# yutongwangBIT/multi_orbslam3

Measured on AMD Instinct MI355X. Metric: tracking+localBA frames/sec (aggregate over agents; 1 agent per GPU), higher is better.
Workload: dtype u8/int32 (ORB front-end, Hamming), f64 (local BA)

## Files before the change

### include/orbgpu.h

```cpp
#ifndef ORBGPU_H_
#define ORBGPU_H_

#include <stdint.h>

#ifdef __cplusplus
extern "C" {
#endif

enum {
  ORBG_OK = 0,
  ORBG_EMPTY = -1,
  ORBG_BAD_ARG = -2,
  ORBG_CAP_EXCEEDED = -3,
  ORBG_HIP_ERROR = -4,
  ORBG_NO_DEVICE = -5,
  ORBG_INTERNAL = -6
};

enum {
  LBA_APPLIED = 0,
  LBA_ABORTED_BEFORE_OPT = 1,
  LBA_REJECTED_OUTLIERS = 2
};

// ... 609 lines not shown
int lba_solve(const lba_problem* p, const volatile int32_t* stop_flag, lba_result* r);
int lba_solve_b(const lba_problem* p, const volatile uint8_t* stop_bool, lba_result* r);

typedef struct lba_handle lba_handle;
int lba_create(int device, int cap_poses, int cap_points, int cap_edges, lba_handle** out);
int lba_destroy(lba_handle* h);
int lba_solve_h(lba_handle* h, const lba_problem* p, const volatile int32_t* stop_flag, lba_result* r);
int lba_solve_hb(lba_handle* h, const lba_problem* p, const volatile uint8_t* stop_bool, lba_result* r);
int lba_solve_async(lba_handle* h, const lba_problem* problem, const volatile int32_t* stop_flag, lba_result* result);
int lba_solve_async_b(lba_handle* h, const lba_problem* problem, const volatile uint8_t* stop_bool, lba_result* result);
int lba_wait(lba_handle* h, double* solve_ms );
int lba_set_profiling(lba_handle* h, int on, int reset);
int lba_get_solver_stats(lba_handle* h, double* sum_ms, int64_t* n_brackets, int32_t* n_unknowns, int32_t* matrix_core);
int lba_event_overhead(lba_handle* h, int reps, float* ms);
int lba_get_watchdog_count(lba_handle* h, int64_t* n_timeouts);


typedef struct pose_opt_problem {
  int32_t n;
  const float* Xw;
  const float* u;
  const float* v;
  const float* ur;
  const float* inv_sigma2;
  float fx, fy, cx, cy, bf;
  float Tcw[16];
  int32_t device;
  const orbg_camera_rig* rig;
} pose_opt_problem;

// ... 43 lines not shown
```

### multi_orbslam3_amd/_capi.py

```python
import ctypes as C
import os

import numpy as np

_HERE = os.path.dirname(os.path.abspath(__file__))
LIB_PATH = os.environ.get("ORBG_LIB") or os.path.join(_HERE, "liborbgpu.so")

ORBG_OK, ORBG_EMPTY, ORBG_BAD_ARG, ORBG_CAP_EXCEEDED, ORBG_HIP_ERROR, ORBG_NO_DEVICE, ORBG_INTERNAL = 0, -1, -2, -3, -4, -5, -6
LBA_APPLIED, LBA_ABORTED_BEFORE_OPT, LBA_REJECTED_OUTLIERS = 0, 1, 2
GRID_COLS, GRID_ROWS = 64, 48

u8p = C.POINTER(C.c_uint8)
i32p = C.POINTER(C.c_int32)
u32p = C.POINTER(C.c_uint32)
f32p = C.POINTER(C.c_float)
f64p = C.POINTER(C.c_double)

KEYPOINT_DTYPE = np.dtype([("x", "<f4"), ("y", "<f4"), ("size", "<f4"), ("angle", "<f4"),
                           ("response", "<f4"), ("octave", "<i4")])
EDGE_DTYPE = np.dtype([("pose", "<i4"), ("point", "<i4"), ("u", "<f4"), ("v", "<f4"), ("ur", "<f4"),
                       ("inv_sigma2", "<f4")])
assert KEYPOINT_DTYPE.itemsize == 24 and EDGE_DTYPE.itemsize == 24


# ... 240 lines not shown


EXPORTED_SYMBOLS = [
    "orbx_create", "orbx_destroy", "orbx_get_tables", "orbx_extract", "orbx_extract_stereo",
    "orbx_extract_stereo_dev", "orbx_get_level", "orbx_get_level_bordered", "orbx_get_candidates", "orbx_stereo_match",
    "orbm_frame_create", "orbm_frame_destroy", "orbm_frame_upload", "orbm_frame_from_extractor", "orbx_frame_stereo_dev", "orbx_frame_stereo", "orbx_frame_stereo_dev_submit", "orbx_frame_stereo_dev_wait", "orbx_frame_stereo_submit", "orbx_frame_stereo_wait", "orbx_set_frame_outputs",
    "orbm_frame_get_grid", "orbm_hamming_matrix", "orbm_hamming_best2", "orbm_is_in_frustum",
    "orbm_search_by_projection_mps", "orbm_is_in_frustum_rig", "orbm_search_by_projection_mps_rig", "orbm_search_by_projection_frame_rig", "orbm_search_by_bow_rig", "orbx_fisheye_stereo_matches", "orbm_map_create", "orbm_map_destroy", "orbm_map_upload",
    "orbm_search_local_points", "orbm_search_local_points_vis", "orbm_search_by_projection_frame", "orbm_search_by_bow",
    "orbm_search_by_projection_sim3", "orbm_search_by_bow_kf",
    "orbv_vocab_create", "orbv_vocab_destroy", "orbv_text_load", "orbv_text_view", "orbv_text_free", "orbv_vocab_from_text", "orbv_transform", "orbv_transform_frame", "orbv_bow_assemble",
    "orbm_distinctive_descriptors", "orbv_score_l1", "orbk_wire_bytes", "orbk_pack_frame", "orbk_frame_from_wire",
    "orbm_frame_download",
    "lba_solve", "lba_create", "lba_destroy", "lba_solve_h", "lba_solve_async", "lba_wait", "pose_optimize",
    "lba_solve_b", "lba_solve_hb", "lba_solve_async_b",
    "lba_set_profiling", "lba_get_solver_stats", "lba_event_overhead", "lba_get_watchdog_count",
    "orbd_database_create", "orbd_database_destroy", "orbd_detect_n_best_candidates",
    "orbx_set_stream", "orbm_frame_set_stream", "orbm_map_set_stream", "lba_set_stream", "orbv_vocab_set_stream", "orbd_database_set_stream",
    "pose_opt_set_stream", "orbx_get_ctor_timeline", "orbm_map_set_observations", "orbm_search_by_projection_reloc", "orbm_search_by_projection_reloc_cam", "orbm_search_by_projection_sim3_cam", "orbm_lastview_create", "orbm_lastview_destroy", "orbm_lastview_upload",
    "orbm_search_by_projection_frame_resident", "orbg_quiesce", "orbg_set_wait_policy", "orbg_get_wait_policy",
    "orbx_frame_mono", "orbx_frame_mono_dev", "orbx_frame_mono_submit", "orbx_frame_mono_dev_submit", "orbx_frame_mono_wait",
    "orbx_set_frame_outputs_un", "orbx_undistort_points",
    "orbx_frame_rgbd", "orbx_frame_rgbd_dev", "orbx_frame_rgbd_submit", "orbx_frame_rgbd_dev_submit", "orbx_frame_rgbd_wait",
    "orbx_depth_at_points",
    "orbm_sim3_create", "orbm_sim3_destroy", "orbm_sim3_set_stream", "orbm_sim3_set_problem", "orbm_sim3_set_ransac_parameters",
    "orbm_sim3_ransac_iterations", "orbm_sim3_resolve_draws", "orbm_sim3_iterate", "orbm_sim3_solve_batch",
    "orbm_sim3_optimize", "orbm_sim3_optimize_batch",
    "orbm_create_new_points", "orbm_search_for_triangulation", "orbm_fuse", "orbm_search_for_initialization",
    "orbg_version", "orbg_strerror", "orbg_device_count", "orbx_get_timings", "orbx_event_overhead", "orbx_set_profile_interval", "orbx_set_profile_kernel", "orbx_get_fast_kernel_stats", "orbx_set_profiling",
]

# ... 61 lines not shown
```

### multi_orbslam3_amd/csrc/lba.hip

```cpp

#include <time.h>

#include <condition_variable>
#include <atomic>
#include <unistd.h>
#include <mutex>
#include <thread>

#include "common.hpp"
#include "wave.hpp"

#include <algorithm>
#include <cmath>
#include <limits>
#include <numeric>
#include <type_traits>

using namespace orbg;

#include "ldlt_mfma.hpp"
#include "ldlt_xcd.hpp"
#include "se3.hpp"

using namespace orbg_se3;

namespace {

#ifdef LBA_PROFILE
__device__ long long g_lba_prof[3][8 + 2 * 1020];
#define LBA_PROF_BEGIN(kern) const int lbp_k = (kern); const long long lbp_t0 = (long long)wall_clock64(); \
  if (threadIdx.x == 0 && blockIdx.x < 1020) g_lba_prof[lbp_k][8 + 2 * blockIdx.x] = lbp_t0
#define LBA_PROF_END() do { if (threadIdx.x == 0 && blockIdx.x < 1020) g_lba_prof[lbp_k][9 + 2 * blockIdx.x] = (long long)wall_clock64(); } while (0)
#define LBA_PROF_PHASE(block, slot) do { if (threadIdx.x == 0 && (int)blockIdx.x == (block)) g_lba_prof[lbp_k][slot] = (long long)wall_clock64() - lbp_t0; } while (0)
#else
#define LBA_PROF_BEGIN(kern) do { } while (0)
#define LBA_PROF_END() do { } while (0)
// ... 722 lines not shown
__device__ inline void inv3_sym(const double* h6, double lambda, double* o) {
  const double m0 = h6[0] + lambda, m1 = h6[1], m2 = h6[2], m4 = h6[3] + lambda, m5 = h6[4], m8 = h6[5] + lambda;
  const double c00 = m4 * m8 - m5 * m5, c01 = m5 * m2 - m1 * m8, c02 = m1 * m5 - m4 * m2;
  const double det = m0 * c00 + m1 * c01 + m2 * c02;
  const double id = 1.0 / det;
  o[0] = c00 * id; o[1] = c01 * id; o[2] = c02 * id;
  o[3] = o[1]; o[4] = (m0 * m8 - m2 * m2) * id; o[5] = (m2 * m1 - m0 * m5) * id;
  o[6] = o[2]; o[7] = o[5]; o[8] = (m0 * m4 - m1 * m1) * id;
}

struct PairItem { int ea, eb, l; };

constexpr int kSchurThreads = 256;

constexpr int kSortPfThreads = 64, kSortPfCap = 64;
template <int NT, int CAP, bool BY_EDGE = false>
__device__ __forceinline__ void sort_pf_block(int bid, int nL, const int* __restrict__ pf_start, int* __restrict__ pf_edges,
                                              int* __restrict__ pf_col, unsigned long long* __restrict__ lm_mask,
                                              const lba_edge* __restrict__ edges, const int* __restrict__ pose_col) {
  __shared__ int s_e[NT][CAP + 1];
  __shared__ int s_c[NT][CAP + 1];
  const int l = bid * NT + threadIdx.x;
  if (l >= nL) return;
  const int b0 = pf_start[l], cnt = pf_start[l + 1] - b0;
  unsigned long long m = 0;
  if (cnt <= CAP) {
    int* const se = s_e[threadIdx.x];
    int* const sc = s_c[threadIdx.x];
    for (int j = 0; j < cnt; j++) se[j] = pf_edges[b0 + j];
    for (int j = 0; j < cnt; j++) sc[j] = pose_col[edges[se[j]].pose];
    for (int a2 = 1; a2 < cnt; a2++) {
      const int e = se[a2], key = sc[a2];
      int b2 = a2 - 1;
      while (b2 >= 0 && (sc[b2] > key || (BY_EDGE && sc[b2] == key && se[b2] > e))) { se[b2 + 1] = se[b2]; sc[b2 + 1] = sc[b2]; b2--; }
      se[b2 + 1] = e; sc[b2 + 1] = key;
    }
    for (int j = 0; j < cnt; j++) { pf_edges[b0 + j] = se[j]; pf_col[b0 + j] = sc[j]; m |= 1ull << sc[j]; }
  } else {
    for (int a2 = b0 + 1; a2 < b0 + cnt; a2++) {
      const int e = pf_edges[a2], key = pose_col[edges[e].pose];
      int b2 = a2 - 1;
      while (b2 >= b0 && (pose_col[edges[pf_edges[b2]].pose] > key ||
                          (BY_EDGE && pose_col[edges[pf_edges[b2]].pose] == key && pf_edges[b2] > e))) { pf_edges[b2 + 1] = pf_edges[b2]; b2--; }
      pf_edges[b2 + 1] = e;
    }
    for (int j = b0; j < b0 + cnt; j++) { const int c = pose_col[edges[pf_edges[j]].pose]; pf_col[j] = c; m |= 1ull << c; }
  }
  lm_mask[l] = m;
}

__global__ __launch_bounds__(256) void k_csr_fill(int n_edges, const lba_edge* __restrict__ edges, const int* __restrict__ pose_col,
                                                 const int* __restrict__ point_col, int* __restrict__ cur_pt, int* __restrict__ cur_ps,
                                                 int* __restrict__ cur_pf, int* __restrict__ pt_edges, int* __restrict__ ps_edges,
                                                 int* __restrict__ pf_edges) {
  __shared__ int s_cnt[64], s_base[64];
  const int k = blockIdx.x * 256 + threadIdx.x;
  if (threadIdx.x < 64) s_cnt[threadIdx.x] = 0;
  __syncthreads();
  int lc = -1, pc = -1, my = 0;
  if (k < n_edges) {
    const lba_edge e = edges[k];
    lc = point_col[e.point]; pc = pose_col[e.pose];
    pt_edges[atomicAdd(&cur_pt[lc], 1)] = k;
    if (pc >= 0) { pf_edges[atomicAdd(&cur_pf[lc], 1)] = k; my = atomicAdd(&s_cnt[pc], 1); }
  }
  __syncthreads();
  if (threadIdx.x < 64 && s_cnt[threadIdx.x] > 0) s_base[threadIdx.x] = atomicAdd(&cur_ps[threadIdx.x], s_cnt[threadIdx.x]);
  __syncthreads();
  if (pc >= 0) ps_edges[s_base[pc] + my] = k;
}
constexpr int kPrep256Cap = 16, kPrep256Pad = 8, kPrep256Zero = 4;
constexpr int kCsrPoseCap = 4096, kCsrPtCap = 16;
__global__ __launch_bounds__(256) void k_csr_sort(int nP, int nL, const int* __restrict__ ps_start, int* __restrict__ ps_edges,
                                                 const int* __restrict__ pt_start, int* __restrict__ pt_edges,
                                                 const int* __restrict__ pf_start, int* __restrict__ pf_edges, int* __restrict__ pf_col,
                                                 unsigned long long* __restrict__ lm_mask, const lba_edge* __restrict__ edges,
                                                 const int* __restrict__ pose_col, int n_unknowns, double* __restrict__ St,
                                                 double* __restrict__ xzero, int n_zero) {
  __shared__ int s_pose[kCsrPoseCap];
  __shared__ int s_pt[256][kCsrPtCap + 1];
  int bid = (int)blockIdx.x;
  const int tid = threadIdx.x;
  if (bid < nP) {
    const int b0 = ps_start[bid], cnt = ps_start[bid + 1] - b0;
    int m = 1;
    while (m < cnt) m <<= 1;
    for (int i = tid; i < m; i += 256) s_pose[i] = i < cnt ? ps_edges[b0 + i] : 0x7FFFFFFF;
    __syncthreads();
    for (int k2 = 2; k2 <= m; k2 <<= 1)
      for (int j = k2 >> 1; j > 0; j >>= 1) {
        for (int i = tid; i < m; i += 256) {
          const int ixj = i ^ j;
          if (ixj > i) {
            const int a = s_pose[i], c = s_pose[ixj];
            const bool up = (i & k2) == 0;
            if ((a > c) == up) { s_pose[i] = c; s_pose[ixj] = a; }
          }
        }
        __syncthreads();
      }
    for (int i = tid; i < cnt; i += 256) ps_edges[b0 + i] = s_pose[i];
    return;
  }
  bid -= nP;
  const int n_pt_blocks = (nL + 255) / 256;
  if (bid < n_pt_blocks) {
    const int l = bid * 256 + tid;
    if (l < nL) {
      const int b0 = pt_start[l], cnt = pt_start[l + 1] - b0;
      if (cnt <= kCsrPtCap) {
        int* const se = s_pt[tid];
        for (int j = 0; j < cnt; j++) se[j] = pt_edges[b0 + j];
        for (int a2 = 1; a2 < cnt; a2++) {
          const int e = se[a2];
          int b2 = a2 - 1;
          while (b2 >= 0 && se[b2] > e) { se[b2 + 1] = se[b2]; b2--; }
          se[b2 + 1] = e;
        }
        for (int j = 0; j < cnt; j++) pt_edges[b0 + j] = se[j];
      } else {
        for (int a2 = b0 + 1; a2 < b0 + cnt; a2++) {
          const int e = pt_edges[a2];
          int b2 = a2 - 1;
          while (b2 >= b0 && pt_edges[b2] > e) { pt_edges[b2 + 1] = pt_edges[b2]; b2--; }
          pt_edges[b2 + 1] = e;
        }
      }
    }
    sort_pf_block<256, kCsrPtCap, true>(bid, nL, pf_start, pf_edges, pf_col, lm_mask, edges, pose_col);
    return;
  }
  bid -= n_pt_blocks;
  if (bid < kPrep256Pad) { if (St) ldltm::image_pad_range(n_unknowns, St, bid * 256 + tid, kPrep256Pad * 256); return; }
  bid -= kPrep256Pad;
  for (int i = bid * 256 + tid; i < n_zero; i += kPrep256Zero * 256) xzero[i] = 0.0;
}

template <class CamT>
__global__ __launch_bounds__(256) void k_errlin_prep(int n_errlin_blocks, int n_sort_blocks, int* __restrict__ pf_edges_w, int* __restrict__ pf_col_w,
                                                    const int* __restrict__ pf_start, unsigned long long* __restrict__ lm_mask,
                                                    int n_unknowns, double* __restrict__ St, double* __restrict__ xzero, int n_zero,
                                                    int nP, int n_edges, const lba_edge* __restrict__ edges, const PoseQ* __restrict__ poses,
                                               const double* __restrict__ points, CamT c, Huber hb, double* __restrict__ err,
                                               double* __restrict__ chi2, const int* __restrict__ pose_col,
                                               const int* __restrict__ point_col, double* __restrict__ EB,
                                               const int* __restrict__ ps_start, const int* __restrict__ ps_edges,
                                               double* __restrict__ Hpp, double* __restrict__ bp, double* __restrict__ partial,
                                               unsigned* __restrict__ ticket, const double* __restrict__ scale_partial, int n_scale_partial,
                                               const int* __restrict__ ok_flag, HostRec* __restrict__ rec, unsigned seq, int n_edge_blocks,
                                               int nL, const int* __restrict__ pt_start, const int* __restrict__ pt_edges,
// ... 480 lines not shown
  if (blockIdx.x == 0)
    finish_block(n_partial, partial, nP, nL, nullptr, bp, bl, Hpp, Hll, 0.0, nullptr, 0, 1, rec, lambda_init, lambda0_out);
  else
    build_items_block((int)blockIdx.x - 1, nP, nL, lm_mask, pf_start, pf_edges, pf_col, items, cap, pair_count);
}

}


struct StopRef {
  const volatile int32_t* i32 = nullptr;
  const volatile uint8_t* u8 = nullptr;
};
struct LbaSwitches {
  bool ldlt_wide = false;
  int ldlt_xcd = 1;
  bool ldlt_xcd_short_once = false;
  static LbaSwitches from_env() {
    LbaSwitches w;
    w.ldlt_wide = getenv("ORBG_LDLT_WIDE") != nullptr;
    if (const char* e = getenv("ORBG_LDLT_XCD")) { w.ldlt_xcd = !strcmp(e, "0") ? 0 : !strcmp(e, "safe") ? 2 : 1; w.ldlt_xcd_short_once = !strcmp(e, "short"); }
    return w;
  }
};
struct LinSet {
  DevBuf<double> EB, Hll, bl, Hpp, bp;
  int reserve(int NE, int nL, int nP) {
    int rc;
    if ((rc = EB.reserve(std::max<size_t>((size_t)NE * kEB, 1))) || (rc = Hll.reserve(std::max<size_t>(6 * (size_t)nL, 1))) ||
        (rc = bl.reserve(std::max<size_t>(3 * (size_t)nL, 1))) || (rc = Hpp.reserve(std::max<size_t>(21 * (size_t)nP, 1))) ||
        (rc = bp.reserve(std::max<size_t>(6 * (size_t)nP, 1))))
      return rc;
    return ORBG_OK;
  }
  void release() { EB.release(); Hll.release(); bl.release(); Hpp.release(); bp.release(); }
// ... 17 lines not shown
  DevBuf<double> d_err, d_chi2, d_partial, d_S, d_bs, d_x;
  LinSet lin[2];
  DevBuf<double> d_lambda0;
  DevBuf<double> d_wide;
  DevBuf<double> d_St, d_wfac;
  DevBuf<int> d_ok;
  PinnedBuf<HostRec> rec;
  unsigned rec_seq = 0;
  PinnedBuf<uint8_t> up_h, dl_h;
  DevBuf<uint8_t> up_d;
  DevBuf<double> d_scale_partial;
  DevBuf<unsigned> d_ticket;
  StreamSignal sig;
  std::vector<int> s_pose_deg, s_point_deg, s_pose_col, s_point_col, s_pf_deg, s_f1, s_f2, s_f3, s_fill, s_row_off, s_junk;
  std::vector<unsigned> s_cnt4;
  int prof_on = 0;
  hipEvent_t prof_ev[2] = {nullptr, nullptr};
  double prof_sum_ms = 0; long long prof_n = 0; int prof_n_unknowns = 0;
  long long prof_solves = 0;
  std::thread worker;
  std::mutex mu;
  std::condition_variable cv;
  std::atomic<bool> quit{false};
  std::atomic<int> job_state{0};
  const lba_problem* job_p = nullptr; StopRef job_stop; lba_result* job_r = nullptr;
  int job_status = ORBG_OK;
  double job_ms = 0;
};

extern "C" int lba_create(int device, int cap_poses, int cap_points, int cap_edges, lba_handle** out) {
// ... 87 lines not shown
  StopRef ref;
  int trials_done = 0;
  bool past_precheck = false;
  bool operator()() const {
    if (ref.u8) return *ref.u8 != 0;
    if (!ref.i32) return false;
    const int v = *ref.i32;
    if (v == INT32_MIN) return past_precheck;
    return v > 0 || (v < 0 && trials_done >= -v);
  }
};

struct Arena {
  PoseQ* poses; double* points;
  int *pose_col, *point_col, *pt_start, *ps_start, *pf_start;
  int *cur_pt, *cur_ps, *cur_pf;
  int *pt_edges, *ps_edges, *pf_edges, *pf_col;
  unsigned long long* lm_mask;
  int *pair_i1, *pair_i2, *pair_start;
  PairItem* items;
};
struct LbaStructure {
  int NP = 0, NX = 0, NE = 0;
  int nP = 0, nL = 0;
  int n = 0, n_zero = 0;
  int n_blocks_e = 0;
  int n_pairs_all = 0, item_cap = 0;
  int runs = 0;
  int n_right_edges = 0;
  std::vector<uint8_t> rig_secondary;
  bool dev_items = false;
  bool dev_lists = false;
  bool dev_csr = false;
  size_t o_poses = 0, o_points = 0, o_pose_col = 0, o_point_col = 0, o_pt_start = 0, o_ps_start = 0, o_pf_start = 0, o_cur_pt = 0,
         o_cur_ps = 0, o_cur_pf = 0, o_pt_edges = 0, o_ps_edges = 0, o_pf_edges = 0, o_pf_col = 0, o_lm_mask = 0, o_pair_i1 = 0,
         o_pair_i2 = 0, o_pair_start = 0, o_items = 0, o_end = 0;
  size_t off_a = 0;
  Arena H{};
  Arena at(uint8_t* B) const {
    auto I = [B](size_t o) { return reinterpret_cast<int*>(B + o); };
    return Arena{reinterpret_cast<PoseQ*>(B + o_poses), reinterpret_cast<double*>(B + o_points), I(o_pose_col), I(o_point_col),
                 I(o_pt_start), I(o_ps_start), I(o_pf_start), I(o_cur_pt), I(o_cur_ps), I(o_cur_pf), I(o_pt_edges), I(o_ps_edges),
                 I(o_pf_edges), I(o_pf_col), reinterpret_cast<unsigned long long*>(B + o_lm_mask), I(o_pair_i1), I(o_pair_i2),
                 I(o_pair_start), reinterpret_cast<PairItem*>(B + o_items)};
  }
};

struct LmState {
  int version = 0;
  int cur = 0;
  int ls = 0;
  bool err_valid = false;
  bool spec_ready = false;
  int fin_version = -1, solve_version = -1, exp_version = -1, exp_buf = -1;
  double lambda = -1, ni = 2, currentChi = 0;
  int nBad = 0;
  bool first_chi = true;
// ... 150 lines not shown
    return h->rec.h->ok == ldltx::kOkTimedOut ? kRcLdltTimedOut : ORBG_OK;
  }

  int edge_pass() {
    int rc;
    std::vector<int>& pose_deg = h->s_pose_deg; std::vector<int>& point_deg = h->s_point_deg;
    std::vector<int>& pf_raw = h->s_f3;
    pose_deg.assign(NP, 0); point_deg.assign(NX, 0); pf_raw.assign(NX, 0);
    if ((rc = h->edges_pin.reserve(std::max(NE, 1))) || (rc = h->d_edges.reserve(std::max(NE, 1)))) return rc;
    lba_edge* const edges = h->edges_pin.h;
    unsigned prev_pt = ~0u;
    if (NE < 65536) {
      std::vector<unsigned>& cnt4 = h->s_cnt4;
      cnt4.assign(4 * (size_t)NX, 0u);
      unsigned* const c4 = cnt4.data();
      int* const pd = pose_deg.data();
      const uint8_t* const fixed = p->pose_fixed;
      for (int k = 0; k < NE; k++) {
        const lba_edge e = p->edges[k];
        edges[k] = e;
        const unsigned ep = (unsigned)e.pose, ex = (unsigned)e.point;
        if (ep >= (unsigned)NP || ex >= (unsigned)NX) return ORBG_BAD_ARG;
        pd[ep]++;
        c4[(size_t)(k & 3) * NX + ex] += 1u + ((fixed[ep] ? 0u : 1u) << 16);
        runs += ex != prev_pt;
        prev_pt = ex;
      }
      int* const pdeg = point_deg.data(); int* const pfr = pf_raw.data();
      for (int i = 0; i < NX; i++) {
        const unsigned sum = c4[i] + c4[(size_t)NX + i] + c4[2 * (size_t)NX + i] + c4[3 * (size_t)NX + i];
        pdeg[i] = (int)(sum & 0xFFFFu); pfr[i] = (int)(sum >> 16);
      }
    } else {
      for (int k = 0; k < NE; k++) {
        const lba_edge e = p->edges[k];
        edges[k] = e;
        const unsigned ep = (unsigned)e.pose, ex = (unsigned)e.point;
        if (ep >= (unsigned)NP || ex >= (unsigned)NX) return ORBG_BAD_ARG;
        pose_deg[ep]++; point_deg[ex]++;
        pf_raw[ex] += p->pose_fixed[ep] ? 0 : 1;
// ... 14 lines not shown
    if (NE > 0) upload16(reinterpret_cast<const uint8_t*>(h->edges_pin.d), reinterpret_cast<uint8_t*>(h->d_edges.p), sizeof(lba_edge) * (size_t)NE, st);
    return ORBG_OK;
  }
  int layout() {
    constexpr bool kRig = std::is_same<CamT, CamRig>::value;
    const std::vector<int>& pose_deg = h->s_pose_deg; const std::vector<int>& point_deg = h->s_point_deg;
    const std::vector<int>& pf_raw = h->s_f3;
    std::vector<int>& pose_col_v = h->s_pose_col; std::vector<int>& point_col_v = h->s_point_col;
    pose_col_v.assign(NP, -1); point_col_v.assign(NX, -1);
    for (int i = 0; i < NP; i++) if (!p->pose_fixed[i] && pose_deg[i] > 0) pose_col_v[i] = nP++;
    for (int i = 0; i < NX; i++) if (point_deg[i] > 0) point_col_v[i] = nL++;
    n = 6 * nP; n_zero = n + 3 * nL;
    n_blocks_e = (NE + 255) / 256;
    std::vector<int>& pf_deg = h->s_pf_deg; std::vector<int>& pt_cnt = h->s_f1; std::vector<int>& ps_cnt = h->s_f2;
    pf_deg.assign(nL + 1, 0); pt_cnt.assign(nL + 1, 0); ps_cnt.assign(nP + 1, 0);
    int n_free_edges = 0;
    for (int i = 0; i < NX; i++) { const int lc = point_col_v[i]; if (lc >= 0) { pt_cnt[lc] = point_deg[i]; pf_deg[lc] = pf_raw[i]; } }
    for (int i = 0; i < NP; i++) { const int pc = pose_col_v[i]; if (pc >= 0) { ps_cnt[pc] = pose_deg[i]; n_free_edges += pose_deg[i]; } }
    size_t n_items = 0;
    for (int l = 0; l < nL; l++) n_items += (size_t)pf_deg[l] * (pf_deg[l] + 1) / 2;
    n_pairs_all = nP * (nP + 1) / 2;
    size_t off = 0;
    auto take = [&](size_t bytes) { const size_t o = off; off = (off + bytes + 63) & ~(size_t)63; return o; };
    o_poses = take(sizeof(PoseQ) * (size_t)NP); o_points = take(24 * (size_t)NX);
    o_pose_col = take(4 * (size_t)NP); o_point_col = take(4 * (size_t)NX); o_pt_start = take(4 * ((size_t)nL + 1));
    o_ps_start = take(4 * ((size_t)nP + 1)); o_pf_start = take(4 * ((size_t)nL + 1));
    o_cur_pt = take(4 * (size_t)nL); o_cur_ps = take(4 * (size_t)nP); o_cur_pf = take(4 * (size_t)nL);
    o_pt_edges = take(4 * (size_t)NE); o_ps_edges = take(4 * (size_t)n_free_edges);
    o_pf_edges = take(4 * (size_t)n_free_edges); o_pf_col = take(4 * (size_t)n_free_edges);
    int max_pose_edges = 1;
    for (int i = 0; i < nP; i++) max_pose_edges = std::max(max_pose_edges, ps_cnt[i]);
    item_cap = std::min(std::max(nL, 1), max_pose_edges);
    dev_items = nP >= 1 && nP <= 64 && (size_t)n_pairs_all * (size_t)item_cap * sizeof(PairItem) <= ((size_t)64 << 20);
    dev_lists = dev_items && nP >= 1 && ldltm::supports(6 * nP);
    dev_csr = dev_lists && NE > 0 && nL > 0 && max_pose_edges <= kCsrPoseCap && NE >= 16384 && !kRig;
    o_lm_mask = take(8 * (size_t)nL);
    o_pair_i1 = take(4 * (size_t)n_pairs_all); o_pair_i2 = take(4 * (size_t)n_pairs_all); o_pair_start = take(4 * ((size_t)n_pairs_all + 1));
    o_items = take(dev_items ? 0 : sizeof(PairItem) * n_items);
    o_end = off;
    off_a = dev_csr ? o_pt_edges : dev_lists ? o_pf_col : o_pf_edges;
    int rc;
    if ((rc = h->up_h.reserve(off + 64)) || (rc = h->up_d.reserve(off + 64))) return rc;
    H = at(h->up_h.h);
    return ORBG_OK;
  }
  void fill_lists() {
    constexpr bool kRig = std::is_same<CamT, CamRig>::value;
    const Arena A = H;
    const lba_edge* const edges = h->edges_pin.h;
    memcpy(A.pose_col, h->s_pose_col.data(), 4 * (size_t)NP);
    memcpy(A.point_col, h->s_point_col.data(), 4 * (size_t)NX);
    const std::vector<int>& pt_cnt = h->s_f1; const std::vector<int>& ps_cnt = h->s_f2; const std::vector<int>& pf_deg = h->s_pf_deg;
    A.pt_start[0] = 0; A.pf_start[0] = 0; A.ps_start[0] = 0;
    for (int i = 0; i < nL; i++) { A.pt_start[i + 1] = A.pt_start[i] + pt_cnt[i]; A.pf_start[i + 1] = A.pf_start[i] + pf_deg[i]; }
    for (int i = 0; i < nP; i++) A.ps_start[i + 1] = A.ps_start[i] + ps_cnt[i];
    if (dev_csr) {
      memcpy(A.cur_pt, A.pt_start, 4 * (size_t)nL); memcpy(A.cur_ps, A.ps_start, 4 * (size_t)nP); memcpy(A.cur_pf, A.pf_start, 4 * (size_t)nL);
      return;
    }
    std::vector<int>& f1 = h->s_f1; std::vector<int>& f2 = h->s_f2; std::vector<int>& f3 = h->s_f3;
    if (runs == nL && !kRig) {
      f2.assign(A.ps_start, A.ps_start + nP);
      f2.push_back(0);
      std::vector<int>& junk = h->s_junk;
      if ((int)junk.size() < NE + 1) junk.resize((size_t)NE + 1);
      int* const ps_base[2] = {junk.data(), A.ps_edges};
      int* const f2p = f2.data();
      int prev = -1, pt_pos = 0, pf_pos = 0;
      for (int k = 0; k < NE; k++) {
        const int ex = edges[k].point, lc = A.point_col[ex], pc = A.pose_col[edges[k].pose];
        const bool ch = ex != prev;
        prev = ex;
// ... 60 lines not shown
    if (use_wide && (rc = h->d_wide.reserve(2 * (size_t)n + 32))) return rc;
    if (use_mfma) {
      if ((rc = h->d_St.reserve(ldltm::tile_image_doubles(n))) || (rc = h->d_wfac.reserve(ldltm::wglob_doubles(ldltm::make_geo(n))))) return rc;
    }
    use_xcd = use_mfma && h->sw.ldlt_xcd != 0 && ldltx::pays(n);
    if (use_xcd && !h->ldlt_x.scr) {
      if ((rc = h->d_xscr.reserve(ldltx::scratch_doubles())) || (rc = h->d_xflags.reserve(ldltx::kFlagWords))) return rc;
      ORBG_HIP(hipMemsetAsync(h->d_xflags.p, 0, ldltx::kFlagWords * sizeof(unsigned), st));
      ORBG_HIP(hipMemsetAsync(h->d_xscr.p + ldltx::kGbOff, 0, (ldltx::kWOff - ldltx::kGbOff) * sizeof(double), st));
      h->ldlt_x.bind(h->d_xscr.p, h->d_xflags.p);
      static std::atomic<int> n_users{0};
      h->ldlt_x.pick = ((int)getpid() + n_users.fetch_add(1)) & 7;
    }
    n_blocks_u = (NP + NX + kUpdThreads - 1) / kUpdThreads;
    if ((rc = h->d_scale_partial.reserve(std::max(n_blocks_u, 1)))) return rc;
    if (!h->d_ticket.p) {
      if ((rc = h->d_ticket.reserve(4))) return rc;
      ORBG_HIP(hipMemsetAsync(h->d_ticket.p, 0, 4 * sizeof(unsigned), st));
    }
    size_t off = 0;
    auto take = [&](size_t bytes) { const size_t o = off; off = (off + bytes + 63) & ~(size_t)63; return o; };
    o_rposes = take(sizeof(PoseQ) * (size_t)NP); o_rpoints = take(24 * (size_t)NX); o_rflags = take((size_t)NE);
    o_rchi = take(r->edge_chi2 ? 8 * (size_t)NE : 0);
    if ((rc = h->dl_h.reserve(off + 64))) return rc;
    out.flags = h->dl_h.d + o_rflags;
    out.chi2 = r->edge_chi2 ? reinterpret_cast<double*>(h->dl_h.d + o_rchi) : (double*)nullptr;
    out.poses = reinterpret_cast<PoseQ*>(h->dl_h.d + o_rposes);
    out.points = reinterpret_cast<double*>(h->dl_h.d + o_rpoints);
    prof_this_solve = h->prof_on && (h->prof_solves++ & 3) == 0;
    return ORBG_OK;
  }

  int first_linearisation() {
    first2 = dev_lists && NE > 0 && nL > 0 && !stop();
    if (first2 || !stop()) {
      const int set = lm.ls ^ 1;
      if (first2) {
        if (dev_csr) {
          hipLaunchKernelGGL(k_csr_fill, dim3(n_blocks_e), dim3(256), 0, st, NE, d_edges, D.pose_col, D.point_col, D.cur_pt, D.cur_ps,
                             D.cur_pf, D.pt_edges, D.ps_edges, D.pf_edges);
          const int n_blocks_l = (nL + 255) / 256;
          hipLaunchKernelGGL(k_csr_sort, dim3(nP + n_blocks_l + kPrep256Pad + kPrep256Zero), dim3(256), 0, st, nP, nL, D.ps_start,
                             D.ps_edges, D.pt_start, D.pt_edges, D.pf_start, D.pf_edges, D.pf_col, D.lm_mask, d_edges, D.pose_col, n,
                             use_mfma ? h->d_St.p : (double*)nullptr, h->d_x.p, n_zero);
          errlin(lm.cur, set, false, LmIn{});
        } else {
          errlin_prep(lm.cur, set);
        }
        finish_items(set);
        lm.fin_version = lm.version;
      } else if (NE > 0) {
        errlin(lm.cur, set, false, LmIn{});
        finish_lambda_init(set);
        lm.fin_version = lm.version;
      }
      ORBG_HIP(hipGetLastError());
      lm.err_valid = true;
      lm.spec_ready = true;
    }
    if (first2) return ORBG_OK;
    if (dev_lists) {
      const int nsb = (nL + kSortPfThreads - 1) / kSortPfThreads;
      hipLaunchKernelGGL(k_prep, dim3(nsb + 32 + 8), dim3(kSortPfThreads), 0, st, nsb, nL, D.pf_start, D.pf_edges, D.pf_col, D.lm_mask,
// ... 28 lines not shown
          for (int j = b0; j < e0; j++) m |= 1ull << A.pf_col[j];
          A.lm_mask[l] = m;
        } else {
          for (int a2 = b0; a2 < e0; a2++) {
            const int ro = row_off[A.pf_col[a2]] + 1;
            for (int b2 = a2; b2 < e0; b2++) A.pair_start[ro + A.pf_col[b2]]++;
          }
        }
      }
    }
    for (int i1 = 0, id = 0; i1 < nP; i1++)
      for (int i2 = i1; i2 < nP; i2++, id++) { A.pair_i1[id] = i1; A.pair_i2[id] = i2; }
    int rc;
    if (dev_items) {
      if (stop()) return ORBG_OK;
      if (!dev_lists && (rc = upload_arena(h, off_a, o_pair_start, st))) return rc;
      if (nL > 0 && !first2)
        hipLaunchKernelGGL(k_build_items, dim3(n_pairs_all), dim3(256), 0, st, nP, nL, D.lm_mask, D.pf_start, D.pf_edges, D.pf_col,
                           h->d_items_dev.p, item_cap, h->d_pair_count.p);
      ORBG_HIP(hipGetLastError());
      return ORBG_OK;
    }
    for (int i = 0; i < n_pairs_all; i++) A.pair_start[i + 1] += A.pair_start[i];
    std::vector<int>& fill = h->s_fill;
    fill.assign(A.pair_start, A.pair_start + n_pairs_all);
    const std::vector<int>& row_off = h->s_row_off;
    for (int l = 0; l < nL; l++) {
      const int b0 = A.pf_start[l], e0 = A.pf_start[l + 1];
      for (int a2 = b0; a2 < e0; a2++) {
        const int ro = row_off[A.pf_col[a2]], ea = A.pf_edges[a2];
        for (int b2 = a2; b2 < e0; b2++) A.items[fill[ro + A.pf_col[b2]]++] = PairItem{ea, A.pf_edges[b2], l};
// ... 244 lines not shown

#ifdef LBA_PROFILE
extern "C" int lba_debug_prof(long long* out , int reset) {
  if (hipMemcpyFromSymbol(out, HIP_SYMBOL(g_lba_prof), sizeof(g_lba_prof)) != hipSuccess) return -1;
  if (reset) { static long long z[3][8 + 2 * 1020]; if (hipMemcpyToSymbol(HIP_SYMBOL(g_lba_prof), z, sizeof(z)) != hipSuccess) return -1; }
  return 0;
}
#endif

extern "C" int lba_get_watchdog_count(lba_handle* h, int64_t* n_timeouts) {
  if (!h || !n_timeouts) return ORBG_BAD_ARG;
  *n_timeouts = h->xcd_timeouts;
  return ORBG_OK;
}

extern "C" int lba_event_overhead(lba_handle* h, int reps, float* ms) {
  if (!h || !ms || reps < 1) return ORBG_BAD_ARG;
  int rc = select_device(h->device);
  if (rc) return rc;
  if ((rc = lba_set_profiling(h, h->prof_on, 0))) return rc;
  if (!h->prof_ev[0]) { ORBG_HIP(hipEventCreate(&h->prof_ev[0])); ORBG_HIP(hipEventCreate(&h->prof_ev[1])); }
  double acc = 0;
  for (int i = 0; i < reps; i++) {
    ORBG_HIP(hipEventRecord(h->prof_ev[0], h->stream));
    ORBG_HIP(hipEventRecord(h->prof_ev[1], h->stream));
    ORBG_HIP(hipStreamSynchronize(h->stream));
    float e = 0;
    ORBG_HIP(hipEventElapsedTime(&e, h->prof_ev[0], h->prof_ev[1]));
    acc += e;
  }
// ... 108 lines not shown
```

Baseline: 9059.

## Build LBA CSR edge lists deterministically via per-block pose bases instead of atomics+sort

Replaces the atomic-scatter CSR fill plus bitonic/insertion sort kernels with a single ordered kernel. Host counting now records per-256-edge-block pose counts and each point's first edge, so ps_edges are placed by wave ballot ranks and pt/pf edges are written as contiguous runs. This removes the sort passes and atomics and widens the device-CSR path to smaller problems (NE<65536, edges grouped by point), at the cost of extra host-side counting and a per-block×pose base table upload. Adds a debug API to read back the lists and an env switch to force host lists.

```diff
diff --git a/include/orbgpu.h b/include/orbgpu.h
--- a/include/orbgpu.h
+++ b/include/orbgpu.h
@@ -647,6 +647,13 @@
 int lba_get_solver_stats(lba_handle* h, double* sum_ms, int64_t* n_brackets, int32_t* n_unknowns, int32_t* matrix_core);
 int lba_event_overhead(lba_handle* h, int reps, float* ms);
 int lba_get_watchdog_count(lba_handle* h, int64_t* n_timeouts);
+typedef struct lba_lists_info {
+  int32_t struct_size;
+  int32_t n_free_poses, n_active_points, n_edges, n_free_edges;
+  int32_t device_filled;
+} lba_lists_info;
+int lba_debug_lists(lba_handle* h, lba_lists_info* info, int32_t* pt_start, int32_t* pt_edges, int32_t* ps_start, int32_t* ps_edges,
+                    int32_t* pf_start, int32_t* pf_edges);
 
 
 typedef struct pose_opt_problem {
diff --git a/multi_orbslam3_amd/_capi.py b/multi_orbslam3_amd/_capi.py
--- a/multi_orbslam3_amd/_capi.py
+++ b/multi_orbslam3_amd/_capi.py
@@ -278,7 +278,7 @@
     "orbm_frame_download",
     "lba_solve", "lba_create", "lba_destroy", "lba_solve_h", "lba_solve_async", "lba_wait", "pose_optimize",
     "lba_solve_b", "lba_solve_hb", "lba_solve_async_b",
-    "lba_set_profiling", "lba_get_solver_stats", "lba_event_overhead", "lba_get_watchdog_count",
+    "lba_set_profiling", "lba_get_solver_stats", "lba_event_overhead", "lba_get_watchdog_count", "lba_debug_lists",
     "orbd_database_create", "orbd_database_destroy", "orbd_detect_n_best_candidates",
     "orbx_set_stream", "orbm_frame_set_stream", "orbm_map_set_stream", "lba_set_stream", "orbv_vocab_set_stream", "orbd_database_set_stream",
     "pose_opt_set_stream", "orbx_get_ctor_timeline", "orbm_map_set_observations", "orbm_search_by_projection_reloc", "orbm_search_by_projection_reloc_cam", "orbm_search_by_projection_sim3_cam", "orbm_lastview_create", "orbm_lastview_destroy", "orbm_lastview_upload",
diff --git a/multi_orbslam3_amd/csrc/csr_blocks.hpp b/multi_orbslam3_amd/csrc/csr_blocks.hpp
--- /dev/null
+++ b/multi_orbslam3_amd/csrc/csr_blocks.hpp
@@ -0,0 +1,39 @@
+#pragma once
+#include <cstddef>
+
+namespace orbg {
+namespace csr {
+
+constexpr int kBlockEdges = 256;
+constexpr int kBlockShift = 8;
+
+inline int n_blocks(int n_edges) { return (n_edges + kBlockEdges - 1) / kBlockEdges; }
+inline size_t count_words(int n_edges, int n_poses) { return (size_t)n_blocks(n_edges) * (size_t)n_poses; }
+
+inline void count_edge(int k, unsigned pose, unsigned point, bool new_run, int n_poses, int n_points, int* blk_cnt, int* first_raw) {
+  blk_cnt[(size_t)(k >> kBlockShift) * n_poses + pose]++;
+  first_raw[new_run ? point : (unsigned)n_points] = k;
+}
+
+inline void block_bases(int n_blk, int n_poses, const int* blk_cnt, const int* pose_col, const int* ps_start, int* blk_base) {
+  for (int i = 0; i < n_poses; i++) {
+    const int pc = pose_col[i];
+    int run = pc >= 0 ? ps_start[pc] : 0;
+    for (int b = 0; b < n_blk; b++) {
+      const size_t at = (size_t)b * n_poses + i;
+      const int c = blk_cnt[at];
+      blk_base[at] = pc >= 0 ? run : c;
+      run += c;
+    }
+  }
+}
+
+inline void first_by_column(int n_points, const int* point_col, const int* first_raw, int* first_edge) {
+  for (int i = 0; i < n_points; i++) {
+    const int lc = point_col[i];
+    if (lc >= 0) first_edge[lc] = first_raw[i];
+  }
+}
+
+}
+}
diff --git a/multi_orbslam3_amd/csrc/lba.hip b/multi_orbslam3_amd/csrc/lba.hip
--- a/multi_orbslam3_amd/csrc/lba.hip
+++ b/multi_orbslam3_amd/csrc/lba.hip
@@ -20,6 +20,7 @@
 
 #include "ldlt_mfma.hpp"
 #include "ldlt_xcd.hpp"
+#include "csr_blocks.hpp"
 #include "se3.hpp"
 
 using namespace orbg_se3;
@@ -772,7 +773,7 @@
 constexpr int kSchurThreads = 256;
 
 constexpr int kSortPfThreads = 64, kSortPfCap = 64;
-template <int NT, int CAP, bool BY_EDGE = false>
+template <int NT, int CAP>
 __device__ __forceinline__ void sort_pf_block(int bid, int nL, const int* __restrict__ pf_start, int* __restrict__ pf_edges,
                                               int* __restrict__ pf_col, unsigned long long* __restrict__ lm_mask,
                                               const lba_edge* __restrict__ edges, const int* __restrict__ pose_col) {
@@ -790,7 +791,7 @@
     for (int a2 = 1; a2 < cnt; a2++) {
       const int e = se[a2], key = sc[a2];
       int b2 = a2 - 1;
-      while (b2 >= 0 && (sc[b2] > key || (BY_EDGE && sc[b2] == key && se[b2] > e))) { se[b2 + 1] = se[b2]; sc[b2 + 1] = sc[b2]; b2--; }
+      while (b2 >= 0 && sc[b2] > key) { se[b2 + 1] = se[b2]; sc[b2 + 1] = sc[b2]; b2--; }
       se[b2 + 1] = e; sc[b2 + 1] = key;
     }
     for (int j = 0; j < cnt; j++) { pf_edges[b0 + j] = se[j]; pf_col[b0 + j] = sc[j]; m |= 1ull << sc[j]; }
@@ -798,8 +799,7 @@
     for (int a2 = b0 + 1; a2 < b0 + cnt; a2++) {
       const int e = pf_edges[a2], key = pose_col[edges[e].pose];
       int b2 = a2 - 1;
-      while (b2 >= b0 && (pose_col[edges[pf_edges[b2]].pose] > key ||
-                          (BY_EDGE && pose_col[edges[pf_edges[b2]].pose] == key && pf_edges[b2] > e))) { pf_edges[b2 + 1] = pf_edges[b2]; b2--; }
+      while (b2 >= b0 && pose_col[edges[pf_edges[b2]].pose] > key) { pf_edges[b2 + 1] = pf_edges[b2]; b2--; }
       pf_edges[b2 + 1] = e;
     }
     for (int j = b0; j < b0 + cnt; j++) { const int c = pose_col[edges[pf_edges[j]].pose]; pf_col[j] = c; m |= 1ull << c; }
@@ -807,91 +807,49 @@
   lm_mask[l] = m;
 }
 
-__global__ __launch_bounds__(256) void k_csr_fill(int n_edges, const lba_edge* __restrict__ edges, const int* __restrict__ pose_col,
-                                                 const int* __restrict__ point_col, int* __restrict__ cur_pt, int* __restrict__ cur_ps,
-                                                 int* __restrict__ cur_pf, int* __restrict__ pt_edges, int* __restrict__ ps_edges,
-                                                 int* __restrict__ pf_edges) {
-  __shared__ int s_cnt[64], s_base[64];
-  const int k = blockIdx.x * 256 + threadIdx.x;
-  if (threadIdx.x < 64) s_cnt[threadIdx.x] = 0;
-  __syncthreads();
-  int lc = -1, pc = -1, my = 0;
-  if (k < n_edges) {
-    const lba_edge e = edges[k];
-    lc = point_col[e.point]; pc = pose_col[e.pose];
-    pt_edges[atomicAdd(&cur_pt[lc], 1)] = k;
-    if (pc >= 0) { pf_edges[atomicAdd(&cur_pf[lc], 1)] = k; my = atomicAdd(&s_cnt[pc], 1); }
-  }
-  __syncthreads();
-  if (threadIdx.x < 64 && s_cnt[threadIdx.x] > 0) s_base[threadIdx.x] = atomicAdd(&cur_ps[threadIdx.x], s_cnt[threadIdx.x]);
-  __syncthreads();
-  if (pc >= 0) ps_edges[s_base[pc] + my] = k;
-}
 constexpr int kPrep256Cap = 16, kPrep256Pad = 8, kPrep256Zero = 4;
-constexpr int kCsrPoseCap = 4096, kCsrPtCap = 16;
-__global__ __launch_bounds__(256) void k_csr_sort(int nP, int nL, const int* __restrict__ ps_start, int* __restrict__ ps_edges,
-                                                 const int* __restrict__ pt_start, int* __restrict__ pt_edges,
-                                                 const int* __restrict__ pf_start, int* __restrict__ pf_edges, int* __restrict__ pf_col,
-                                                 unsigned long long* __restrict__ lm_mask, const lba_edge* __restrict__ edges,
-                                                 const int* __restrict__ pose_col, int n_unknowns, double* __restrict__ St,
-                                                 double* __restrict__ xzero, int n_zero) {
-  __shared__ int s_pose[kCsrPoseCap];
-  __shared__ int s_pt[256][kCsrPtCap + 1];
-  int bid = (int)blockIdx.x;
-  const int tid = threadIdx.x;
-  if (bid < nP) {
-    const int b0 = ps_start[bid], cnt = ps_start[bid + 1] - b0;
-    int m = 1;
-    while (m < cnt) m <<= 1;
-    for (int i = tid; i < m; i += 256) s_pose[i] = i < cnt ? ps_edges[b0 + i] : 0x7FFFFFFF;
+__global__ __launch_bounds__(256) void k_csr_ordered(int n_edges, int n_edge_blocks, int n_poses, int nL, const lba_edge* __restrict__ edges,
+                                                    const int* __restrict__ pose_col, const int* __restrict__ blk_base,
+                                                    const int* __restrict__ first_edge, const int* __restrict__ pt_start,
+                                                    const int* __restrict__ pf_start, int* __restrict__ pt_edges,
+                                                    int* __restrict__ ps_edges, int* __restrict__ pf_edges ,
+                                                    unsigned* __restrict__ ticket) {
+  __shared__ int s_wcnt[4][64];
+  const int bid = (int)blockIdx.x, tid = (int)threadIdx.x, lane = tid & 63, wv = tid >> 6;
+  if (bid < n_edge_blocks) {
+    if (bid == 0 && tid < 4) ticket[tid] = 0u;
+    s_wcnt[wv][lane] = 0;
+    const int k = bid * 256 + tid;
+    int pose = -1, pc = -1;
+    if (k < n_edges) { pose = edges[k].pose; pc = pose_col[pose]; }
+    int rank = 0;
+    unsigned long long todo = __ballot(pc >= 0);
+    while (todo) {
+      const int leader = __ffsll((long long)todo) - 1;
+      const int lp = __builtin_amdgcn_readlane(pc, leader);
+      const unsigned long long same = __ballot(pc == lp);
+      if (pc == lp) {
+        rank = __popcll(same & ((1ull << lane) - 1ull));
+        if (lane == leader) s_wcnt[wv][lp] = __popcll(same);
+      }
+      todo &= ~same;
+    }
     __syncthreads();
-    for (int k2 = 2; k2 <= m; k2 <<= 1)
-      for (int j = k2 >> 1; j > 0; j >>= 1) {
-        for (int i = tid; i < m; i += 256) {
-          const int ixj = i ^ j;
-          if (ixj > i) {
-            const int a = s_pose[i], c = s_pose[ixj];
-            const bool up = (i & k2) == 0;
-            if ((a > c) == up) { s_pose[i] = c; s_pose[ixj] = a; }
-          }
-        }
-        __syncthreads();
-      }
-    for (int i = tid; i < cnt; i += 256) ps_edges[b0 + i] = s_pose[i];
+    if (pc >= 0) {
+      int before = 0;
+      for (int w = 0; w < wv; w++) before += s_wcnt[w][pc];
+      ps_edges[blk_base[(size_t)bid * n_poses + pose] + before + rank] = k;
+    }
     return;
   }
-  bid -= nP;
-  const int n_pt_blocks = (nL + 255) / 256;
-  if (bid < n_pt_blocks) {
-    const int l = bid * 256 + tid;
-    if (l < nL) {
-      const int b0 = pt_start[l], cnt = pt_start[l + 1] - b0;
-      if (cnt <= kCsrPtCap) {
-        int* const se = s_pt[tid];
-        for (int j = 0; j < cnt; j++) se[j] = pt_edges[b0 + j];
-        for (int a2 = 1; a2 < cnt; a2++) {
-          const int e = se[a2];
-          int b2 = a2 - 1;
-          while (b2 >= 0 && se[b2] > e) { se[b2 + 1] = se[b2]; b2--; }
-          se[b2 + 1] = e;
-        }
-        for (int j = 0; j < cnt; j++) pt_edges[b0 + j] = se[j];
-      } else {
-        for (int a2 = b0 + 1; a2 < b0 + cnt; a2++) {
-          const int e = pt_edges[a2];
-          int b2 = a2 - 1;
-          while (b2 >= b0 && pt_edges[b2] > e) { pt_edges[b2 + 1] = pt_edges[b2]; b2--; }
-          pt_edges[b2 + 1] = e;
-        }
-      }
-    }
-    sort_pf_block<256, kCsrPtCap, true>(bid, nL, pf_start, pf_edges, pf_col, lm_mask, edges, pose_col);
-    return;
-  }
-  bid -= n_pt_blocks;
-  if (bid < kPrep256Pad) { if (St) ldltm::image_pad_range(n_unknowns, St, bid * 256 + tid, kPrep256Pad * 256); return; }
-  bid -= kPrep256Pad;
-  for (int i = bid * 256 + tid; i < n_zero; i += kPrep256Zero * 256) xzero[i] = 0.0;
+  const int l = (bid - n_edge_blocks) * 256 + tid;
+  if (l >= nL) return;
+  const int k0 = first_edge[l], b0 = pt_start[l], cnt = pt_start[l + 1] - b0;
+  int q = pf_start[l];
+  for (int j = 0; j < cnt; j++) {
+    pt_edges[b0 + j] = k0 + j;
+    if (pf_edges && pose_col[edges[k0 + j].pose] >= 0) pf_edges[q++] = k0 + j;
+  }
 }
 
 template <class CamT>
@@ -1402,11 +1360,13 @@
 };
 struct LbaSwitches {
   bool ldlt_wide = false;
+  bool host_lists = false;
   int ldlt_xcd = 1;
   bool ldlt_xcd_short_once = false;
   static LbaSwitches from_env() {
     LbaSwitches w;
     w.ldlt_wide = getenv("ORBG_LDLT_WIDE") != nullptr;
+    if (const char* e = getenv("ORBG_LBA_HOST_LISTS")) w.host_lists = strcmp(e, "0") != 0;
     if (const char* e = getenv("ORBG_LDLT_XCD")) { w.ldlt_xcd = !strcmp(e, "0") ? 0 : !strcmp(e, "safe") ? 2 : 1; w.ldlt_xcd_short_once = !strcmp(e, "short"); }
     return w;
   }
@@ -1454,6 +1414,8 @@
   StreamSignal sig;
   std::vector<int> s_pose_deg, s_point_deg, s_pose_col, s_point_col, s_pf_deg, s_f1, s_f2, s_f3, s_fill, s_row_off, s_junk;
   std::vector<unsigned> s_cnt4;
+  std::vector<int> s_blk_cnt, s_first_raw;
+  struct { int nP = 0, nL = 0, NE = 0, n_free_edges = 0, device_filled = 0; size_t o_pt_start = 0, o_ps_start = 0, o_pf_start = 0, o_pt_edges = 0, o_ps_edges = 0, o_pf_edges = 0; } lists;
   int prof_on = 0;
   hipEvent_t prof_ev[2] = {nullptr, nullptr};
   double prof_sum_ms = 0; long long prof_n = 0; int prof_n_unknowns = 0;
@@ -1571,7 +1533,7 @@
 struct Arena {
   PoseQ* poses; double* points;
   int *pose_col, *point_col, *pt_start, *ps_start, *pf_start;
-  int *cur_pt, *cur_ps, *cur_pf;
+  int *first_edge, *blk_base;
   int *pt_edges, *ps_edges, *pf_edges, *pf_col;
   unsigned long long* lm_mask;
   int *pair_i1, *pair_i2, *pair_start;
@@ -1589,15 +1551,16 @@
   bool dev_items = false;
   bool dev_lists = false;
   bool dev_csr = false;
-  size_t o_poses = 0, o_points = 0, o_pose_col = 0, o_point_col = 0, o_pt_start = 0, o_ps_start = 0, o_pf_start = 0, o_cur_pt = 0,
-         o_cur_ps = 0, o_cur_pf = 0, o_pt_edges = 0, o_ps_edges = 0, o_pf_edges = 0, o_pf_col = 0, o_lm_mask = 0, o_pair_i1 = 0,
+  int n_free_edges = 0;
+  size_t o_poses = 0, o_points = 0, o_pose_col = 0, o_point_col = 0, o_pt_start = 0, o_ps_start = 0, o_pf_start = 0, o_first_edge = 0,
+         o_blk_base = 0, o_pt_edges = 0, o_ps_edges = 0, o_pf_edges = 0, o_pf_col = 0, o_lm_mask = 0, o_pair_i1 = 0,
          o_pair_i2 = 0, o_pair_start = 0, o_items = 0, o_end = 0;
   size_t off_a = 0;
   Arena H{};
   Arena at(uint8_t* B) const {
     auto I = [B](size_t o) { return reinterpret_cast<int*>(B + o); };
     return Arena{reinterpret_cast<PoseQ*>(B + o_poses), reinterpret_cast<double*>(B + o_points), I(o_pose_col), I(o_point_col),
-                 I(o_pt_start), I(o_ps_start), I(o_pf_start), I(o_cur_pt), I(o_cur_ps), I(o_cur_pf), I(o_pt_edges), I(o_ps_edges),
+                 I(o_pt_start), I(o_ps_start), I(o_pf_start), I(o_first_edge), I(o_blk_base), I(o_pt_edges), I(o_ps_edges),
                  I(o_pf_edges), I(o_pf_col), reinterpret_cast<unsigned long long*>(B + o_lm_mask), I(o_pair_i1), I(o_pair_i2),
                  I(o_pair_start), reinterpret_cast<PairItem*>(B + o_items)};
   }
@@ -1778,6 +1741,9 @@
       std::vector<unsigned>& cnt4 = h->s_cnt4;
       cnt4.assign(4 * (size_t)NX, 0u);
       unsigned* const c4 = cnt4.data();
+      h->s_blk_cnt.assign(csr::count_words(NE, NP), 0);
+      if (h->s_first_raw.size() < (size_t)NX + 1) h->s_first_raw.resize((size_t)NX + 1);
+      int* const bc = h->s_blk_cnt.data(); int* const fr = h->s_first_raw.data();
       int* const pd = pose_deg.data();
       const uint8_t* const fixed = p->pose_fixed;
       for (int k = 0; k < NE; k++) {
@@ -1787,7 +1753,9 @@
         if (ep >= (unsigned)NP || ex >= (unsigned)NX) return ORBG_BAD_ARG;
         pd[ep]++;
         c4[(size_t)(k & 3) * NX + ex] += 1u + ((fixed[ep] ? 0u : 1u) << 16);
-        runs += ex != prev_pt;
+        const bool ch = ex != prev_pt;
+        csr::count_edge(k, ep, ex, ch, NP, NX, bc, fr);
+        runs += ch;
         prev_pt = ex;
       }
       int* const pdeg = point_deg.data(); int* const pfr = pf_raw.data();
@@ -1832,7 +1800,7 @@
     n_blocks_e = (NE + 255) / 256;
     std::vector<int>& pf_deg = h->s_pf_deg; std::vector<int>& pt_cnt = h->s_f1; std::vector<int>& ps_cnt = h->s_f2;
     pf_deg.assign(nL + 1, 0); pt_cnt.assign(nL + 1, 0); ps_cnt.assign(nP + 1, 0);
-    int n_free_edges = 0;
+    n_free_edges = 0;
     for (int i = 0; i < NX; i++) { const int lc = point_col_v[i]; if (lc >= 0) { pt_cnt[lc] = point_deg[i]; pf_deg[lc] = pf_raw[i]; } }
     for (int i = 0; i < NP; i++) { const int pc = pose_col_v[i]; if (pc >= 0) { ps_cnt[pc] = pose_deg[i]; n_free_edges += pose_deg[i]; } }
     size_t n_items = 0;
@@ -1843,7 +1811,7 @@
     o_poses = take(sizeof(PoseQ) * (size_t)NP); o_points = take(24 * (size_t)NX);
     o_pose_col = take(4 * (size_t)NP); o_point_col = take(4 * (size_t)NX); o_pt_start = take(4 * ((size_t)nL + 1));
     o_ps_start = take(4 * ((size_t)nP + 1)); o_pf_start = take(4 * ((size_t)nL + 1));
-    o_cur_pt = take(4 * (size_t)nL); o_cur_ps = take(4 * (size_t)nP); o_cur_pf = take(4 * (size_t)nL);
+    o_first_edge = take(4 * (size_t)nL); o_blk_base = take(4 * csr::count_words(NE, NP));
     o_pt_edges = take(4 * (size_t)NE); o_ps_edges = take(4 * (size_t)n_free_edges);
     o_pf_edges = take(4 * (size_t)n_free_edges); o_pf_col = take(4 * (size_t)n_free_edges);
     int max_pose_edges = 1;
@@ -1851,12 +1819,13 @@
     item_cap = std::min(std::max(nL, 1), max_pose_edges);
     dev_items = nP >= 1 && nP <= 64 && (size_t)n_pairs_all * (size_t)item_cap * sizeof(PairItem) <= ((size_t)64 << 20);
     dev_lists = dev_items && nP >= 1 && ldltm::supports(6 * nP);
-    dev_csr = dev_lists && NE > 0 && nL > 0 && max_pose_edges <= kCsrPoseCap && NE >= 16384 && !kRig;
+    dev_csr = dev_items && NE > 0 && NE < 65536 && nL > 0 && runs == nL && !kRig && !h->sw.host_lists;
     o_lm_mask = take(8 * (size_t)nL);
     o_pair_i1 = take(4 * (size_t)n_pairs_all); o_pair_i2 = take(4 * (size_t)n_pairs_all); o_pair_start = take(4 * ((size_t)n_pairs_all + 1));
     o_items = take(dev_items ? 0 : sizeof(PairItem) * n_items);
     o_end = off;
     off_a = dev_csr ? o_pt_edges : dev_lists ? o_pf_col : o_pf_edges;
+    h->lists = {nP, nL, NE, n_free_edges, dev_csr ? 1 : 0, o_pt_start, o_ps_start, o_pf_start, o_pt_edges, o_ps_edges, o_pf_edges};
     int rc;
     if ((rc = h->up_h.reserve(off + 64)) || (rc = h->up_d.reserve(off + 64))) return rc;
     H = at(h->up_h.h);
@@ -1873,7 +1842,14 @@
     for (int i = 0; i < nL; i++) { A.pt_start[i + 1] = A.pt_start[i] + pt_cnt[i]; A.pf_start[i + 1] = A.pf_start[i] + pf_deg[i]; }
     for (int i = 0; i < nP; i++) A.ps_start[i + 1] = A.ps_start[i] + ps_cnt[i];
     if (dev_csr) {
-      memcpy(A.cur_pt, A.pt_start, 4 * (size_t)nL); memcpy(A.cur_ps, A.ps_start, 4 * (size_t)nP); memcpy(A.cur_pf, A.pf_start, 4 * (size_t)nL);
+      csr::block_bases(n_blocks_e, NP, h->s_blk_cnt.data(), A.pose_col, A.ps_start, A.blk_base);
+      csr::first_by_column(NX, A.point_col, h->s_first_raw.data(), A.first_edge);
+      if (!dev_lists)
+        for (int l = 0; l < nL; l++) {
+          int q = A.pf_start[l];
+          for (int k = A.first_edge[l], k1 = k + pt_cnt[l]; k < k1; k++)
+            if (A.pose_col[edges[k].pose] >= 0) A.pf_edges[q++] = k;
+        }
       return;
     }
     std::vector<int>& f1 = h->s_f1; std::vector<int>& f2 = h->s_f2; std::vector<int>& f3 = h->s_f3;
@@ -1964,10 +1940,8 @@
     }
     n_blocks_u = (NP + NX + kUpdThreads - 1) / kUpdThreads;
     if ((rc = h->d_scale_partial.reserve(std::max(n_blocks_u, 1)))) return rc;
-    if (!h->d_ticket.p) {
-      if ((rc = h->d_ticket.reserve(4))) return rc;
-      ORBG_HIP(hipMemsetAsync(h->d_ticket.p, 0, 4 * sizeof(unsigned), st));
-    }
+    if (!h->d_ticket.p && (rc = h->d_ticket.reserve(4))) return rc;
+    if (!dev_csr) ORBG_HIP(hipMemsetAsync(h->d_ticket.p, 0, 4 * sizeof(unsigned), st));
     size_t off = 0;
     auto take = [&](size_t bytes) { const size_t o = off; off = (off + bytes + 63) & ~(size_t)63; return o; };
     o_rposes = take(sizeof(PoseQ) * (size_t)NP); o_rpoints = take(24 * (size_t)NX); o_rflags = take((size_t)NE);
@@ -1983,20 +1957,16 @@
 
   int first_linearisation() {
     first2 = dev_lists && NE > 0 && nL > 0 && !stop();
+    if (dev_csr) {
+      hipLaunchKernelGGL(k_csr_ordered, dim3(n_blocks_e + (nL + 255) / 256), dim3(256), 0, st, NE, n_blocks_e, NP, nL, d_edges,
+                         D.pose_col, D.blk_base, D.first_edge, D.pt_start, D.pf_start, D.pt_edges, D.ps_edges,
+                         dev_lists ? D.pf_edges : (int*)nullptr, h->d_ticket.p);
+      ORBG_HIP(hipGetLastError());
+    }
     if (first2 || !stop()) {
       const int set = lm.ls ^ 1;
       if (first2) {
-        if (dev_csr) {
-          hipLaunchKernelGGL(k_csr_fill, dim3(n_blocks_e), dim3(256), 0, st, NE, d_edges, D.pose_col, D.point_col, D.cur_pt, D.cur_ps,
-                             D.cur_pf, D.pt_edges, D.ps_edges, D.pf_edges);
-          const int n_blocks_l = (nL + 255) / 256;
-          hipLaunchKernelGGL(k_csr_sort, dim3(nP + n_blocks_l + kPrep256Pad + kPrep256Zero), dim3(256), 0, st, nP, nL, D.ps_start,
-                             D.ps_edges, D.pt_start, D.pt_edges, D.pf_start, D.pf_edges, D.pf_col, D.lm_mask, d_edges, D.pose_col, n,
-                             use_mfma ? h->d_St.p : (double*)nullptr, h->d_x.p, n_zero);
-          errlin(lm.cur, set, false, LmIn{});
-        } else {
-          errlin_prep(lm.cur, set);
-        }
+        errlin_prep(lm.cur, set);
         finish_items(set);
         lm.fin_version = lm.version;
       } else if (NE > 0) {
@@ -2055,7 +2025,7 @@
     int rc;
     if (dev_items) {
       if (stop()) return ORBG_OK;
-      if (!dev_lists && (rc = upload_arena(h, off_a, o_pair_start, st))) return rc;
+      if (!dev_lists && (rc = upload_arena(h, dev_csr ? o_pf_edges : off_a, o_pair_start, st))) return rc;
       if (nL > 0 && !first2)
         hipLaunchKernelGGL(k_build_items, dim3(n_pairs_all), dim3(256), 0, st, nP, nL, D.lm_mask, D.pf_start, D.pf_edges, D.pf_col,
                            h->d_items_dev.p, item_cap, h->d_pair_count.p);
@@ -2330,6 +2300,28 @@
   return ORBG_OK;
 }
 
+extern "C" int lba_debug_lists(lba_handle* h, lba_lists_info* info, int32_t* pt_start, int32_t* pt_edges, int32_t* ps_start,
+                               int32_t* ps_edges, int32_t* pf_start, int32_t* pf_edges) {
+  if (!h || !info || info->struct_size != (int32_t)sizeof(lba_lists_info)) return ORBG_BAD_ARG;
+  if (h->job_state.load() != 0) return ORBG_BAD_ARG;
+  const auto& L = h->lists;
+  info->n_free_poses = L.nP; info->n_active_points = L.nL; info->n_edges = L.NE; info->n_free_edges = L.n_free_edges;
+  info->device_filled = L.device_filled;
+  if (!h->up_d.p) return ORBG_OK;
+  int rc = select_device(h->device);
+  if (rc) return rc;
+  ORBG_HIP(hipStreamSynchronize(h->stream));
+  auto get = [&](int32_t* dst, size_t off, size_t count) -> int {
+    if (dst && count) ORBG_HIP(hipMemcpy(dst, h->up_d.p + off, 4 * count, hipMemcpyDeviceToHost));
+    return ORBG_OK;
+  };
+  if ((rc = get(pt_start, L.o_pt_start, (size_t)L.nL + 1)) || (rc = get(pt_edges, L.o_pt_edges, (size_t)L.NE)) ||
+      (rc = get(ps_start, L.o_ps_start, (size_t)L.nP + 1)) || (rc = get(ps_edges, L.o_ps_edges, (size_t)L.n_free_edges)) ||
+      (rc = get(pf_start, L.o_pf_start, (size_t)L.nL + 1)) || (rc = get(pf_edges, L.o_pf_edges, (size_t)L.n_free_edges)))
+    return rc;
+  return ORBG_OK;
+}
+
 extern "C" int lba_event_overhead(lba_handle* h, int reps, float* ms) {
   if (!h || !ms || reps < 1) return ORBG_BAD_ARG;
   int rc = select_device(h->device);
```

Result: slower. 8853 (-2.3%).
